# haoheliu/ssr_eval

Hardware: AMD Instinct MI355X
Metric: utterance-pairs/sec (LSD+SSIM, 48kHz, n_fft=2048) (higher is better)
Workload: dtype f64

## Files before the change

ssr_eval_amd/csrc/ssr_metrics.h:

```cpp
#pragma once
#include "ssr_stft.h"

#define SSR_SSIM_NT 64
#define SSR_SSIM_MAXCPT 6
#define SSR_SSIM_WIN 7

SSR_HD constexpr int ssr_ssim_strip_out(int cpt) { return SSR_SSIM_NT * cpt; }
SSR_HD int ssr_ssim_pick_cpt(int n_bins) {
  const int outs = n_bins - (SSR_SSIM_WIN - 1);
  if (outs <= SSR_SSIM_NT * 4) {
    int c = (outs + SSR_SSIM_NT - 1) / SSR_SSIM_NT;
    return c < 1 ? 1 : c;
  }
  int best = 4, best_waste = 1 << 30;
  for (int c = 4; c <= SSR_SSIM_MAXCPT; ++c) {
    const int w = SSR_SSIM_NT * c;
    const int waste = ((outs + w - 1) / w) * w - outs;
    if (waste < best_waste) { best_waste = waste; best = c; }
  }
  return best;
}

struct SsrSsimParams {
  const float* x;
  const float* y;
  const int64_t* frame_off;
  const int32_t* n_rows;
  int F;
  int rows_per_tile, n_row_tiles, n_strips;
  double* part;
  int pitch;
  int vi_n;
  int64_t x_plane;
};
SSR_DEV int ssr_ssim_pitch(const SsrSsimParams& p) { return p.pitch ? p.pitch : p.F; }

template <int CPT> struct SsrSsimRegs {
  double cs[CPT + 1][4];
  double s;
  float px[2][4][CPT + 1];
  float ring[SSR_SSIM_WIN][CPT + 1];
  double pxy[CPT], pb[CPT];
  float den[CPT];
};

template <int CPT> SSR_DEV int ssr_ssim_slot(int c) { return (CPT % 2 == 0) ? c + c / CPT : c; }
template <int CPT> SSR_DEV int ssr_ssim_slot_of(int tid, int d) { return (CPT % 2 == 0) ? (CPT + 1) * tid + (d + d / CPT) : CPT * tid + d; }

template <int CPT, bool CONTIG = false> struct SsrSsimLds {
  static constexpr int PW = SSR_SSIM_NT * CPT + 8 + ((CPT % 2 == 0) ? (SSR_SSIM_NT * CPT + 8) / CPT + 1 : 0);
  static constexpr int NQ = CONTIG ? 1 : 4;
  static constexpr int RW = SSR_SSIM_NT * CPT + 8;
  static constexpr size_t ring_bytes() { return CONTIG ? sizeof(float) * SSR_SSIM_WIN * RW : 0; }
  static constexpr size_t bytes() { return ring_bytes() + sizeof(double) * (NQ * PW + SSR_SSIM_NT + 16 + 8); }
  float* yring; double* col; double* sc0; double* sc1; double* res;
  SSR_MEMBER explicit SsrSsimLds(char* base) {
    yring = reinterpret_cast<float*>(base);
    col = reinterpret_cast<double*>(base + ring_bytes());
    sc0 = col + NQ * PW;
    sc1 = sc0 + SSR_SSIM_NT;
    res = sc1 + 16;
  }
};

SSR_DEV void ssr_ld4(const float* p, float* o) {
#ifdef SSR_HOST_EMU
  memcpy(o, p, 16);
#else
  typedef float f4 __attribute__((ext_vector_type(4)));
  const f4 v = *reinterpret_cast<const f4*>(p);
  o[0] = v.x; o[1] = v.y; o[2] = v.z; o[3] = v.w;
#endif
}
SSR_DEV void ssr_st4(float* p, const float* v) {
#ifdef SSR_HOST_EMU
  memcpy(p, v, 16);
#else
  typedef float f4 __attribute__((ext_vector_type(4)));
  *reinterpret_cast<f4*>(p) = f4{v[0], v[1], v[2], v[3]};
#endif
}

struct SsrImage {
#ifdef SSR_HOST_EMU
  const float* base;
  SSR_MEMBER SsrImage(const float* p, int64_t) : base(p) {}
  SSR_MEMBER float at(int64_t row_elems, unsigned col) const { return base[row_elems + col]; }
  SSR_MEMBER void at4(int64_t row_elems, unsigned col, float* o) const { memcpy(o, base + row_elems + col, 16); }
#else
  __amdgpu_buffer_rsrc_t rsrc;
  SSR_MEMBER SsrImage(const float* p, int64_t n_elems)
      : rsrc(__builtin_amdgcn_make_buffer_rsrc((void*)p, 0, (int)(n_elems * 4), 0x00020000)) {}
  SSR_MEMBER float at(int64_t row_elems, unsigned col) const {
    return __builtin_bit_cast(float, __builtin_amdgcn_raw_buffer_load_b32(rsrc, (int)(col * 4u), (int)(row_elems * 4), 0));
  }
  SSR_MEMBER void at4(int64_t row_elems, unsigned col, float* o) const {
    typedef float f4 __attribute__((ext_vector_type(4)));
    const f4 v = __builtin_bit_cast(f4, __builtin_amdgcn_raw_buffer_load_b128(rsrc, (int)(col * 4u), (int)(row_elems * 4), 0));
    o[0] = v.x; o[1] = v.y; o[2] = v.z; o[3] = v.w;
  }
#endif
};

template <int CPT, bool CONTIG> SSR_DEV int ssr_ssim_col(int tid, int i) {
  if constexpr (CONTIG) return (i < CPT) ? CPT * tid + i : SSR_SSIM_NT * CPT + tid;
  else return tid + SSR_SSIM_NT * i;
}

SSR_DEV int ssr_ssim_row_ahead(int row, int T) { return row < T ? row : T - 1; }

template <int CPT, bool CONTIG, int SET>
SSR_DEV void ssr_ssim_row_load(const SsrSsimParams& p, SsrSsimRegs<CPT>& R, int tid, const SsrImage& x, const SsrImage& y,
                               int row_add, int row_sub, int c_in0, int ncol_in) {
  constexpr int VC = CPT + 1;
  const bool sub = row_sub >= 0;
  const int pitch = ssr_ssim_pitch(p);
// ... 34 lines not shown
#pragma unroll
  for (int i = 0; i < VC; ++i) {
    if (ssr_ssim_col<CPT, CONTIG>(tid, i) < ncol_in) {
      const double a = (double)R.px[SET][0][i], b = (double)R.px[SET][1][i];
      const double c = sub ? (double)R.px[SET][2][i] : 0.0, d = sub ? (double)R.px[SET][3][i] : 0.0;
      R.cs[i][0] = (R.cs[i][0] + a) - c;
      R.cs[i][1] = (R.cs[i][1] + b) - d;
      R.cs[i][2] = fma(-d, d, fma(-c, c, fma(b, b, fma(a, a, R.cs[i][2]))));
      R.cs[i][3] = fma(-c, d, fma(a, b, R.cs[i][3]));
    }
  }
}

template <int CPT, int SET, int SLOT>
SSR_DEV void ssr_ssim_row_apply_contig(SsrSsimRegs<CPT>& R, float* yrow, int tid) {
  constexpr int VC = CPT + 1;
  float* own = yrow + CPT * tid;
  float* ext = yrow + SSR_SSIM_NT * CPT + (tid < 7 ? tid : 7);
  float d[VC];
#pragma unroll
  for (int h = 0; h < CPT / 4; ++h) ssr_ld4(own + 4 * h, d + 4 * h);
  d[CPT] = *ext;
#pragma unroll
  for (int h = 0; h < CPT / 4; ++h) ssr_st4(own + 4 * h, R.px[SET][1] + 4 * h);
  *ext = R.px[SET][1][CPT];
#pragma unroll
  for (int i = 0; i < VC; ++i) {
    const double a = (double)R.px[SET][0][i], b = (double)R.px[SET][1][i];
    const double c = (double)R.ring[SLOT][i], dd = (double)d[i];
    R.cs[i][0] = (R.cs[i][0] + a) - c;
    R.cs[i][1] = (R.cs[i][1] + b) - dd;
    R.cs[i][2] = fma(-dd, dd, fma(-c, c, fma(b, b, fma(a, a, R.cs[i][2]))));
    R.cs[i][3] = fma(-c, dd, fma(a, b, R.cs[i][3]));
    R.ring[SLOT][i] = R.px[SET][0][i];
    ssr_touch(R.ring[SLOT][i]);
  }
}

struct SsrSsimK {
  static constexpr double n = 49.0;
  static constexpr float cov = (float)(49.0 / 48.0);
  static constexpr float C1n = (float)((0.01 * 2.0) * (0.01 * 2.0) * 49.0 * 49.0), C2n = (float)((0.03 * 2.0) * (0.03 * 2.0) * 49.0 * 49.0);
};
SSR_DEV void ssr_ssim_stage1(double sx, double sy, double& pxy, double& pp) { pxy = sx * sy; pp = fma(sx, sx, sy * sy); }
SSR_DEV float ssr_ssim_stage2f(double pp, double sq) {
  const double t2 = fma(SsrSsimK::n, sq, -pp);
  const float b1 = (float)pp + SsrSsimK::C1n;
  const float b2 = fmaf(SsrSsimK::cov, (float)t2, SsrSsimK::C2n);
  return b1 * b2;
}
SSR_DEV float ssr_ssim_stage3f(double pxy, double sxy, float b12) {
  const double t1 = fma(SsrSsimK::n, sxy, -pxy);
  const float a1 = fmaf(2.0f, (float)pxy, SsrSsimK::C1n);
  const float a2 = fmaf(2.0f * SsrSsimK::cov, (float)t1, SsrSsimK::C2n);
#ifndef SSR_HOST_EMU
  return (a1 * a2) * __builtin_amdgcn_rcpf(b12);
#else
  return (a1 * a2) / b12;
#endif
}
SSR_DEV double ssr_ssim_value(double sx, double sy, double sq, double sxy) {
  double pxy, pp;
  ssr_ssim_stage1(sx, sy, pxy, pp);
  return (double)ssr_ssim_stage3f(pxy, sxy, ssr_ssim_stage2f(pp, sq));
}

#ifndef SSR_HOST_EMU
#define SSR_SSIM_ST(arr, idx, val) (*(volatile __attribute__((address_space(3))) double*)(&(arr)[idx]) = (val))
#define SSR_SSIM_LD(arr, idx) (*(const volatile __attribute__((address_space(3))) double*)(&(arr)[idx]))
#else
#define SSR_SSIM_ST(arr, idx, val) ((arr)[idx] = (val))
#define SSR_SSIM_LD(arr, idx) ((arr)[idx])
#endif
template <int CPT, bool CONTIG, typename BLK>
SSR_BODY void ssr_ssim_body(const SsrSsimParams& p, BLK& blk, int tile, int item, char* lds_base) {
  constexpr int NT = SSR_SSIM_NT, PW = SsrSsimLds<CPT, CONTIG>::PW, VC = CPT + 1, W = SSR_SSIM_WIN;
  using Regs = SsrSsimRegs<CPT>;
  using Lds = SsrSsimLds<CPT, CONTIG>;
  Lds L(lds_base);
  const int row_tile = tile / p.n_strips, strip = tile % p.n_strips;
  const int item_v = item;
  const float* xbase = p.x;
  if (p.vi_n > 0) { xbase += (int64_t)(item / p.vi_n) * p.x_plane; item = item % p.vi_n; }
  const int T = p.n_rows[item];
  const int out_rows = T - (W - 1);
  const int r0 = row_tile * p.rows_per_tile;
  const int r1 = (r0 + p.rows_per_tile < out_rows) ? r0 + p.rows_per_tile : out_rows;
  const int c_in0 = strip * ssr_ssim_strip_out(CPT);
  const int ncol_in = (p.F - c_in0 < NT * CPT + (W - 1)) ? p.F - c_in0 : NT * CPT + (W - 1);
  const int ncol_out = ncol_in - (W - 1);
  double* part = p.part + (int64_t)item_v * p.n_row_tiles * p.n_strips + tile;
  const int pitch = ssr_ssim_pitch(p);
  const SsrImage x(xbase + p.frame_off[item] * pitch, (int64_t)T * pitch);
  const SsrImage y(p.y + p.frame_off[item] * pitch, (int64_t)T * pitch);

  SSR_REGS(Regs, regs, blk);
  if (r0 >= r1 || ncol_out <= 0) {
    SSR_PHASE(blk, regs, if (tid == 0) *part = 0.0);
    return;
  }
  const int n_steps = (W - 1) + (r1 - r0);
#define SSR_SSIM_STEP(s_, SET, SLOT)                                                                                         \
  SSR_PHASE(blk, regs, {                                                                                                    \
    ssr_ssim_row_apply<CPT, false, SET, SLOT>(R, tid, (s_) >= W, ncol_in);                                                   \
    ssr_ssim_row_load<CPT, false, SET>(p, R, tid, x, y, ssr_ssim_row_ahead(r0 + (s_) + 2, T),                               \
                                       ((s_) + 2 >= W) ? r0 + (s_) + 2 - W : -1, c_in0, ncol_in);                           \
    if ((s_) >= W - 1) {                                                                                                    \
      for (int i = 0; i < VC; ++i) {                                                                                        \
        const int c = ssr_ssim_col<CPT, false>(tid, i);                                                                     \
        if (c < ncol_in)                                                                                                    \
          for (int q = 0; q < 4; ++q) L.col[q * PW + ssr_ssim_slot<CPT>(c)] = R.cs[i][q];                                    \
      }                                                                                                                     \
    }                                                                                                                       \
  });                                                                                                                       \
  if ((s_) >= W - 1) {                                                                                                      \
    SSR_PHASE(blk, regs, {                                                                                                  \
      const int j0 = tid * CPT;                                                                                             \
      if (j0 < ncol_out) {                                                                                                  \
        double w[4][CPT];                                      \
        for (int q = 0; q < 4; ++q) {                                                                                       \
          double v[CPT + W - 1];                                                                                            \
          for (int d = 0; d < CPT + W - 1; ++d) {                                                                           \
            int c = j0 + d;                                                                                                 \
            if (c >= ncol_in) c = ncol_in - 1;                                \
            v[d] = L.col[q * PW + ssr_ssim_slot<CPT>(c)];                                                                   \
          }                                                                                                                 \
          double sw = v[0];                                                                                                 \
          for (int d = 1; d < W; ++d) sw += v[d];                                                                           \
          w[q][0] = sw;                                                                                                     \
          for (int i = 1; i < CPT; ++i) {                                                                                   \
            sw += v[i + W - 1] - v[i - 1];                                                                                  \
            w[q][i] = sw;                                                                                                   \
          }                                                                                                                 \
        }                                                                                                                   \
        for (int i = 0; i < CPT; ++i)                                                                                       \
          if (j0 + i < ncol_out) R.s += ssr_ssim_value(w[0][i], w[1][i], w[2][i], w[3][i]);                                  \
      }                                                                                                                     \
    });                                                                                                                     \
  }
  SSR_PHASE(blk, regs, {
    for (int i = 0; i < VC; ++i)
      for (int q = 0; q < 4; ++q) R.cs[i][q] = 0.0;
    R.s = 0.0;
    if constexpr (CONTIG) {
      const float z4[4] = {0.0f, 0.0f, 0.0f, 0.0f};
      for (int k = 0; k < W; ++k) {
        for (int i = 0; i < VC; ++i) R.ring[k][i] = 0.0f;
        for (int h = 0; h < CPT / 4; ++h) ssr_st4(L.yring + k * Lds::RW + CPT * tid + 4 * h, z4);
        L.yring[k * Lds::RW + NT * CPT + (tid & 7)] = 0.0f;
      }
    }
    ssr_ssim_row_load<CPT, CONTIG, 0>(p, R, tid, x, y, r0, -1, c_in0, ncol_in);
    if (n_steps > 1) ssr_ssim_row_load<CPT, CONTIG, 1>(p, R, tid, x, y, r0 + 1, -1, c_in0, ncol_in);
  });
  if constexpr (CONTIG) {
#define SSR_SSIM_STEP_C(s_, SET, SLOT, HORIZ)                                                                                     \
    SSR_WPHASE(blk, regs, {                                                                                                  \
      ssr_ssim_row_apply_contig<CPT, SET, SLOT>(R, L.yring + (SLOT) * Lds::RW, tid);                                              \
      SSR_SCHED_BARRIER();                                                                                                   \
      ssr_ssim_row_load<CPT, true, SET>(p, R, tid, x, y, ssr_ssim_row_ahead(r0 + (s_) + 2, T), -1, c_in0, ncol_in);          \
      SSR_SCHED_BARRIER();    \
    });                                                                                                                      \
    if (HORIZ) {                                                                                                             \
      SSR_UNROLL for (int q = 0; q < 4; ++q) {                                                                               \
        SSR_WPHASE(blk, regs, {              \
                                \
          SSR_UNROLL for (int i = 0; i < (CPT < 6 ? CPT : 6); ++i) SSR_SSIM_ST(L.col, ssr_ssim_slot_of<CPT>(tid, i), R.cs[i][q]);     \
// ... 51 lines not shown
    } while (0);
#undef SSR_SSIM_STEP_T
#undef SSR_SSIM_STEP_K
#undef SSR_SSIM_STEP_C
  } else {
    for (int s0 = 0; s0 < n_steps; s0 += 2) {
      SSR_SSIM_STEP(s0, 0, 0)
      if (s0 + 1 < n_steps) { SSR_SSIM_STEP(s0 + 1, 1, 0) }
    }
  }
#undef SSR_SSIM_STEP
#define SSR_GET_S(q) R.s
  SSR_BLOCK_SUM(blk, regs, NT, 1, L.sc0, L.sc1, L.res, SSR_GET_S);
#undef SSR_GET_S
  SSR_PHASE(blk, regs, if (tid == 0) *part = L.res[0]);
}

struct SsrSpecRedParams {
  const float* x; const float* y;
  const int64_t* frame_off; const int32_t* n_rows;
  int F, metric_mask, rows_per_chunk, n_chunks;
  double* part;
};
struct SsrSpecRedRegs { double acc[7]; double lsd_sum; };
struct SsrSpecRedLds {
  static constexpr int NT = 256;
  static constexpr size_t bytes() { return sizeof(double) * (NT + 16 + 8); }
  double* sc0; double* sc1; double* res;
  SSR_MEMBER explicit SsrSpecRedLds(char* base) {
    sc0 = reinterpret_cast<double*>(base); sc1 = sc0 + NT; res = sc1 + 16;
  }
};

template <typename BLK>
SSR_BODY void ssr_specred_body(const SsrSpecRedParams& p, BLK& blk, int chunk, int item, char* lds_base) {
  constexpr int NT = SsrSpecRedLds::NT;
  SsrSpecRedLds L(lds_base);
  const int T = p.n_rows[item];
  const int t0 = chunk * p.rows_per_chunk;
  const int t1 = (t0 + p.rows_per_chunk < T) ? t0 + p.rows_per_chunk : T;
  const float* x = p.x + p.frame_off[item] * p.F;
  const float* y = p.y + p.frame_off[item] * p.F;
  double* part = p.part + ((int64_t)item * p.n_chunks + chunk) * SSR_NPART;
  const bool want_lsd = p.metric_mask & SSR_M_LSD;
  SSR_REGS(SsrSpecRedRegs, regs, blk);
  SSR_PHASE(blk, regs, for (int q = 0; q < 7; ++q) R.acc[q] = 0.0; R.lsd_sum = 0.0);
  for (int t = t0; t < t1; ++t) {
    SSR_PHASE(blk, regs, {
      R.acc[0] = 0.0;
      for (int k = tid; k < p.F; k += NT)
        ssr_accumulate_metrics(x[(int64_t)t * p.F + k], y[(int64_t)t * p.F + k], p.metric_mask, R.acc);
      L.sc0[tid] = R.acc[0];
    });
    if (want_lsd) {
      SSR_PHASE(blk, regs, if (tid < 16) {
        double s = 0.0;
        for (int i = tid; i < NT; i += 16) s += L.sc0[i];
        L.sc1[tid] = s;
      });
      SSR_PHASE(blk, regs, if (tid == 0) {
        double s = 0.0;
        for (int i = 0; i < 16; ++i) s += L.sc1[i];
        R.lsd_sum += sqrt(s / (double)p.F);
      });
    }
  }
#define SSR_GET_ACC(q) R.acc[(q) + 1]
  SSR_BLOCK_SUM(blk, regs, NT, 6, L.sc0, L.sc1, L.res, SSR_GET_ACC);
#undef SSR_GET_ACC
  SSR_PHASE(blk, regs, if (tid == 0) {
    part[0] = R.lsd_sum;
    for (int q = 0; q < 6; ++q) part[1 + q] = L.res[q];
    part[7] = 0.0;
  });
}

struct SsrFinalizeParams {
  const double* part; int n_chunks;
  const double* ssim_part; int n_tiles;
  const int32_t* n_rows;
  int F, metric_mask, n_items;
  double* out;
  int vi_n, out_keys, out_key0;
};

SSR_DEV double ssr_sispec_from_sums(double sdd, double stt, double sdt) {
  const double EPS = 1e-12;
  const double den = stt + EPS;
  const double alpha = (stt + sdt) / den;
  const double beta = (EPS - sdt) / den;
  const double tt = alpha * alpha * stt;
  double nn = sdd + 2.0 * beta * sdt + beta * beta * stt;
  if (nn < 0.0) nn = 0.0;
  return 10.0 * log10(tt / (nn + EPS) + EPS);
}

SSR_DEV void ssr_finalize_item(const SsrFinalizeParams& p, int item) {
  const double nan_ = NAN;
  const int real = p.vi_n > 0 ? item % p.vi_n : item;
  double* o = p.vi_n > 0 ? p.out + ((int64_t)real * p.out_keys + p.out_key0 + item / p.vi_n) * 4 : p.out + (int64_t)item * 4;
  const int T = p.n_rows[real];
  o[0] = o[1] = o[2] = o[3] = nan_;
  if (p.part) {
    double s[SSR_NPART];
    for (int q = 0; q < SSR_NPART; ++q) s[q] = 0.0;
    for (int c = 0; c < p.n_chunks; ++c)
      for (int q = 0; q < SSR_NPART; ++q) s[q] += p.part[((int64_t)item * p.n_chunks + c) * SSR_NPART + q];
    if (p.metric_mask & SSR_M_LSD) o[0] = s[0] / (double)T;
    if (p.metric_mask & SSR_M_LOG_SISPEC) o[1] = ssr_sispec_from_sums(s[4], s[5], s[6]);
    if (p.metric_mask & SSR_M_SISPEC) o[2] = ssr_sispec_from_sums(s[1], s[2], s[3]);
  }
  if (p.ssim_part && (p.metric_mask & SSR_M_SSIM)) {
    double s = 0.0;
    for (int c = 0; c < p.n_tiles; ++c) s += p.ssim_part[(int64_t)item * p.n_tiles + c];
    o[3] = (T >= SSR_SSIM_WIN && p.F >= SSR_SSIM_WIN) ? s / ((double)(T - 6) * (double)(p.F - 6)) : nan_;
  }
}
```

ssr_eval_amd/csrc/ssr_specred_wave.h:

```cpp
#pragma once
#include "ssr_stft.h"

struct SsrSpecWaveParams {
  const float* x;
  const float* y;
  const int64_t* frame_off;
  const int32_t* n_rows;
  int F, pitch, metric_mask, rows_per_chunk, n_chunks, vi_n;
  int64_t x_plane;
  double* part;
};

struct SsrSpecTgt2 { f2 t, tt, lt; };

__device__ __forceinline__ SsrSpecTgt2 ssr_spec_tgt2(float t0, float t1) {
  const f2 t = f2_make(t0, t1);
  return {t, t * t, ssr_log10f_fast2(t + f2_splat(1e-12f))};
}
__device__ __forceinline__ void ssr_spec_tgt_sums2(const SsrSpecTgt2& y, double* tsum) {
  const double t0 = (double)y.t.x, l0 = (double)y.lt.x, t1 = (double)y.t.y, l1 = (double)y.lt.y;
  tsum[0] += t0 * t0; tsum[1] += l0 * l0;
  tsum[0] += t1 * t1; tsum[1] += l1 * l1;
}
__device__ __forceinline__ void ssr_spec_est2(float e0, float e1, const SsrSpecTgt2& y, double* acc) {
  const f2 EPS2 = f2_splat(1e-12f);
  const f2 e = f2_make(e0, e1);
  const f2 ee = e + EPS2;
  const f2 d = ssr_log10f_fast2(ssr_divf_fast2(y.tt, ee * ee) + EPS2);
  const f2 dd = d * d;
  const f2 le = ssr_log10f_fast2(ee);
  {
    acc[0] += (double)dd.x;
    const double td = (double)y.t.x, d0 = (double)e.x - td;
    acc[1] += d0 * d0; acc[3] += d0 * td;
    const double ld = (double)y.lt.x, l0 = (double)le.x - ld;
    acc[4] += l0 * l0; acc[6] += l0 * ld;
  }
  {
    acc[0] += (double)dd.y;
    const double td = (double)y.t.y, d0 = (double)e.y - td;
    acc[1] += d0 * d0; acc[3] += d0 * td;
    const double ld = (double)y.lt.y, l0 = (double)le.y - ld;
    acc[4] += l0 * l0; acc[6] += l0 * ld;
  }
}

template <int KG>
__device__ __forceinline__ void ssr_specred_wave_body(const SsrSpecWaveParams& p, int chunk, int group_v) {
  const int lane = (int)threadIdx.x;
  const int key0 = (group_v / p.vi_n) * KG, item = group_v % p.vi_n;
  const int T = p.n_rows[item];
  const int t0 = chunk * p.rows_per_chunk;
  const int t1 = (t0 + p.rows_per_chunk < T) ? t0 + p.rows_per_chunk : T;
  const float* x = p.x + (int64_t)key0 * p.x_plane + p.frame_off[item] * (int64_t)p.pitch;
  const float* y = p.y + p.frame_off[item] * (int64_t)p.pitch;
  const int mask = p.metric_mask;
  const bool want_lsd = mask & SSR_M_LSD;
  constexpr int FULL = SSR_M_LSD | SSR_M_SISPEC | SSR_M_LOG_SISPEC;
  const bool fast = (mask & FULL) == FULL;
  double acc[KG][7];
  double lsd_sum[KG];
  double tsum[2] = {0.0, 0.0};
#pragma unroll
  for (int g = 0; g < KG; ++g) {
    lsd_sum[g] = 0.0;
#pragma unroll
    for (int q = 0; q < 7; ++q) acc[g][q] = 0.0;
  }
  const int nq = (p.F + 3) / 4;
  const int nfull = p.F / 4;
  for (int t = t0; t < t1; ++t) {
    const float4* yr = reinterpret_cast<const float4*>(y + (int64_t)t * p.pitch);
#pragma unroll
    for (int g = 0; g < KG; ++g) acc[g][0] = 0.0;
    if (fast) {
      for (int q = lane; q < nfull; q += 64) {
        const float4 yv = yr[q];
        float4 xv[KG];
#pragma unroll
        for (int g = 0; g < KG; ++g) xv[g] = reinterpret_cast<const float4*>(x + (int64_t)g * p.x_plane + (int64_t)t * p.pitch)[q];
        const SsrSpecTgt2 y01 = ssr_spec_tgt2(yv.x, yv.y), y23 = ssr_spec_tgt2(yv.z, yv.w);
        ssr_spec_tgt_sums2(y01, tsum);
        ssr_spec_tgt_sums2(y23, tsum);
#pragma unroll
        for (int g = 0; g < KG; ++g) {
          ssr_spec_est2(xv[g].x, xv[g].y, y01, acc[g]);
          ssr_spec_est2(xv[g].z, xv[g].w, y23, acc[g]);
        }
      }
      if (nfull < nq && lane == nfull % 64) {
        const float4 yv = yr[nfull];
        const int k = 4 * nfull;
        double a7[7];
#pragma unroll
        for (int g = 0; g < KG; ++g) {
          const float4 xv = reinterpret_cast<const float4*>(x + (int64_t)g * p.x_plane + (int64_t)t * p.pitch)[nfull];
          a7[0] = acc[g][0]; a7[1] = acc[g][1]; a7[2] = tsum[0]; a7[3] = acc[g][3]; a7[4] = acc[g][4]; a7[5] = tsum[1]; a7[6] = acc[g][6];
          ssr_accumulate_metrics<true>(xv.x, yv.x, mask, a7);
          if (k + 1 < p.F) ssr_accumulate_metrics<true>(xv.y, yv.y, mask, a7);
          if (k + 2 < p.F) ssr_accumulate_metrics<true>(xv.z, yv.z, mask, a7);
          acc[g][0] = a7[0]; acc[g][1] = a7[1]; acc[g][3] = a7[3]; acc[g][4] = a7[4]; acc[g][6] = a7[6];
          if (g == KG - 1) { tsum[0] = a7[2]; tsum[1] = a7[5]; }
        }
      }
    } else {
      for (int q = lane; q < nq; q += 64) {
        const float4 yv = yr[q];
        const int k = 4 * q;
#pragma unroll
        for (int g = 0; g < KG; ++g) {
          const float4 xv = reinterpret_cast<const float4*>(x + (int64_t)g * p.x_plane + (int64_t)t * p.pitch)[q];
          ssr_accumulate_metrics<true>(xv.x, yv.x, mask, acc[g]);
          if (k + 1 < p.F) ssr_accumulate_metrics<true>(xv.y, yv.y, mask, acc[g]);
          if (k + 2 < p.F) ssr_accumulate_metrics<true>(xv.z, yv.z, mask, acc[g]);
          if (k + 3 < p.F) ssr_accumulate_metrics<true>(xv.w, yv.w, mask, acc[g]);
        }
      }
    }
    if (want_lsd) {
#pragma unroll
      for (int g = 0; g < KG; ++g) lsd_sum[g] += sqrt(ssr_wave_sum<64>(acc[g][0]) / (double)p.F);
    }
  }
  if (fast) {
#pragma unroll
    for (int g = 0; g < KG; ++g) { acc[g][2] = tsum[0]; acc[g][5] = tsum[1]; }
  }
#pragma unroll
  for (int g = 0; g < KG; ++g) {
    double tot[6];
#pragma unroll
    for (int q = 0; q < 6; ++q) tot[q] = ssr_wave_sum<64>(acc[g][1 + q]);
    if (lane == 0) {
      double* part = p.part + (((int64_t)(key0 + g) * p.vi_n + item) * p.n_chunks + chunk) * SSR_NPART;
// ... 8 lines not shown
```

ssr_eval_amd/csrc/tu_metrics.hip:

```cpp
#include "ssr_host.h"
#include "ssr_metrics.h"
#include "ssr_pair_transform.h"

template <int CPT, bool CONTIG>
__global__ __launch_bounds__(SSR_SSIM_NT, (CPT == 8 ? 2 : 1)) void k_ssim(SsrSsimParams p) {
  extern __shared__ __attribute__((aligned(16))) char smem[];
  SsrBlk blk{(int)threadIdx.x};
  const int tiles = p.n_row_tiles * p.n_strips;
  ssr_ssim_body<CPT, CONTIG>(p, blk, blockIdx.x % tiles, blockIdx.x / tiles, smem);
}


__global__ __launch_bounds__(256) void k_specred(SsrSpecRedParams p) {
  extern __shared__ __attribute__((aligned(16))) char smem[];
  SsrBlk blk{(int)threadIdx.x};
  ssr_specred_body(p, blk, blockIdx.x % p.n_chunks, blockIdx.x / p.n_chunks, smem);
}

__global__ __launch_bounds__(64) void k_finalize(SsrFinalizeParams p) {
  const int item = blockIdx.x * 64 + threadIdx.x;
  if (item < p.n_items) ssr_finalize_item(p, item);
}

struct SsimGeom { int rows_per_tile, n_row_tiles, n_strips, cpt; };
static SsimGeom ssim_geom(int max_rows, int n_bins, int n_items, bool aligned_rows) {
  SsimGeom g;
  const int out_rows = max_rows - 6 > 1 ? max_rows - 6 : 1;
  int64_t r = ((int64_t)out_rows * n_items + ssr_target_wgs() - 1) / ssr_target_wgs();
  if (r < 8) r = 8;
  if (r > 128) r = 128;
  if (r > out_rows) r = out_rows;
  g.rows_per_tile = (int)r;
  g.n_row_tiles = ssr_ceil_div(out_rows, g.rows_per_tile);
  g.cpt = ssr_ssim_pick_cpt(n_bins);
  if (aligned_rows && g.cpt != 4) {
    const int outs = n_bins - (SSR_SSIM_WIN - 1);
    if (outs > 0) {
      const int strips4 = ssr_ceil_div(outs, ssr_ssim_strip_out(4)), strips_c = ssr_ceil_div(outs, ssr_ssim_strip_out(g.cpt));
      if (strips4 * 5 * 68 < strips_c * (g.cpt + 1) * 100) g.cpt = 4;
    }
  }
  if (aligned_rows && g.cpt == 4) {
    constexpr int SSR_SSIM_TRIP4 = 3731, SSR_SSIM_TRIP8 = 6371;
    const int outs = n_bins - (SSR_SSIM_WIN - 1);
    if (outs > 0 && ssr_ceil_div(outs, ssr_ssim_strip_out(8)) * SSR_SSIM_TRIP8 < ssr_ceil_div(outs, ssr_ssim_strip_out(4)) * SSR_SSIM_TRIP4)
      g.cpt = 8;
  }
  g.n_strips = n_bins > 6 ? ssr_ceil_div(n_bins - 6, ssr_ssim_strip_out(g.cpt)) : 1;
  return g;
}


struct PairWs {
  SsrPairGeom g;
  SsimGeom sg;
  SsrPairImages im;
  size_t off_part, off_ssim, total;
};
static PairWs pair_ws(const ssr_plan* pl, int n_items, int max_len, int64_t total_rows, bool in64, bool want_mag) {
  PairWs w;
  w.g = ssr_pair_geom(pl, n_items, max_len, in64);
  w.sg = ssim_geom((int)ssr_num_frames(pl, max_len), pl->n_bins, n_items, true);
  w.im = ssr_pair_images_layout(pl, 1, total_rows, in64, want_mag);
  size_t o = w.im.end;
  w.off_part = o; o += ssr_align256((size_t)n_items * w.g.n_chunks * SSR_NPART * sizeof(double));
  w.off_ssim = o; o += ssr_align256((size_t)n_items * w.sg.n_row_tiles * w.sg.n_strips * sizeof(double));
  w.total = o;
  return w;
}

extern "C" size_t ssr_pair_metrics_workspace_bytes_for(const ssr_plan* pl, int n_items, int max_len, int64_t total_rows,
                                                        unsigned metric_mask) {
  if (!pl || n_items <= 0) return 0;
  const bool mag = metric_mask & SSR_METRIC_SSIM;
  const size_t a = pair_ws(pl, n_items, max_len, total_rows, false, mag).total, b = pair_ws(pl, n_items, max_len, total_rows, true, mag).total;
  return (a > b ? a : b) + ssr_align256((size_t)n_items * sizeof(int32_t));
}

extern "C" size_t ssr_pair_metrics_workspace_bytes(const ssr_plan* pl, int n_items, int max_len, int64_t total_rows) {
  return ssr_pair_metrics_workspace_bytes_for(pl, n_items, max_len, total_rows, SSR_METRIC_ALL);
}

template <int CPT, bool CONTIG = false> static int launch_ssim_inst(const SsrSsimParams& p, int grid, hipStream_t s) {
  const size_t lds = SsrSsimLds<CPT, CONTIG>::bytes();
  static thread_local SsrLdsSlot slot;
  if (int rc = ssr_allow_lds((const void*)k_ssim<CPT, CONTIG>, lds, &slot)) return rc;
  hipLaunchKernelGGL((k_ssim<CPT, CONTIG>), dim3(grid), dim3(SSR_SSIM_NT), lds, s, p);
  HIP_TRY(hipGetLastError());
  return SSR_OK;
}

static int launch_ssim(const float* x, const float* y, const int64_t* frame_off, const int32_t* n_rows, int n_items,
                       int F, int pitch, const SsimGeom& g, double* part, hipStream_t s, int vi_n = 0, int64_t x_plane = 0) {
  SsrSsimParams p{x, y, frame_off, n_rows, F, g.rows_per_tile, g.n_row_tiles, g.n_strips, part, pitch, vi_n, x_plane};
  const int grid = n_items * g.n_row_tiles * g.n_strips;
  const bool contig = pitch > 0 && pitch % 4 == 0 && (((uintptr_t)x | (uintptr_t)y) & 15) == 0;
  if (g.cpt == 8) {
    if (!contig) return ssr_fail(SSR_ERR_UNSUPPORTED, "eight-column SSIM geometry on unaligned rows");
    return launch_ssim_inst<8, true>(p, grid, s);
  }
  if (g.cpt == 4 && contig) return launch_ssim_inst<4, true>(p, grid, s);
  switch (g.cpt) {
    case 1: return launch_ssim_inst<1>(p, grid, s);
    case 2: return launch_ssim_inst<2>(p, grid, s);
    case 3: return launch_ssim_inst<3>(p, grid, s);
    case 4: return launch_ssim_inst<4>(p, grid, s);
    case 5: return launch_ssim_inst<5>(p, grid, s);
    case 6: return launch_ssim_inst<6>(p, grid, s);
  }
  return ssr_fail(SSR_ERR_UNSUPPORTED, "bad SSIM geometry");
}

static int launch_finalize(const double* part, int n_chunks, const double* ssim_part, int n_tiles, const int32_t* n_rows,
                           int F, unsigned mask, int n_items, double* out, hipStream_t s) {
  SsrFinalizeParams p{part, n_chunks, ssim_part, n_tiles, n_rows, F, (int)mask, n_items, out};
  hipLaunchKernelGGL(k_finalize, dim3(ssr_ceil_div(n_items, 64)), dim3(64), 0, s, p);
  HIP_TRY(hipGetLastError());
  return SSR_OK;
}

__global__ void k_rows_from_len(const int32_t* len, int n_items, int n_fft, int hop, int32_t* rows) {
  const int i = blockIdx.x * 256 + threadIdx.x;
  if (i < n_items) rows[i] = ssr_num_frames_dev(len[i], n_fft, hop);
}
int ssr_launch_rows_from_len(const ssr_plan* pl, const int32_t* len, int n_items, int32_t* rows, hipStream_t s) {
  hipLaunchKernelGGL(k_rows_from_len, dim3(ssr_ceil_div(n_items, 256)), dim3(256), 0, s, len, n_items, pl->n_fft, pl->hop, rows);
  HIP_TRY(hipGetLastError());
  return SSR_OK;
}

static int pair_metrics_impl(const ssr_plan* pl, const float* est, const double* est64, const int64_t* est_off,
                             const float* tgt, const double* tgt64, const int64_t* tgt_off, const int32_t* len, const int64_t* frame_off,
                             int n_items, int max_len, int64_t total_rows, unsigned mask, double* out,
                             void* workspace, size_t workspace_bytes, void* stream, int stages) {
  int max_T;
  if (int rc = ssr_check_pair_batch(pl, (est || est64) && (tgt || tgt64) && est_off && tgt_off && len && frame_off && out, n_items, 1, max_len,
                                    mask & SSR_METRIC_SSIM, &max_T))
    return rc;
  if (!max_T) return SSR_OK;
  if ((mask & ~SSR_METRIC_ALL) || mask == 0) return ssr_fail(SSR_ERR_INVALID_ARG, "bad metric mask");
  const bool want_ssim = mask & SSR_METRIC_SSIM;
  if (want_ssim && (max_T < 7 || pl->n_bins < 7)) return ssr_fail(SSR_ERR_INVALID_ARG, "win_size exceeds image extent");
  const PairWs w = pair_ws(pl, n_items, max_len, total_rows, est64 != nullptr, want_ssim);
  const size_t rows_bytes = ssr_align256((size_t)n_items * sizeof(int32_t));
  if (!workspace || workspace_bytes < w.total + rows_bytes) return ssr_fail(SSR_ERR_WORKSPACE, "workspace too small");
  char* ws = (char*)workspace;
  int32_t* rows = (int32_t*)(ws + w.total);
  float *est_plane = (float*)(ws + w.im.off_est), *tgt_plane = (float*)(ws + w.im.off_tgt);
  hipStream_t s = (hipStream_t)stream;
  int rc = SSR_OK;
  if (stages & 1) {
    if ((rc = ssr_launch_rows_from_len(pl, len, n_items, rows, s))) return rc;
    rc = ssr_pair_transform(pl, {len, frame_off, n_items, w.g},
                            {est, est64, est_off, tgt, tgt64, tgt_off, mask, want_ssim ? SSR_OUT_MAG : SSR_OUT_NONE, est_plane, tgt_plane,
                             (double*)(ws + w.off_part)}, s);
    if (rc) return rc;
  }
  if ((stages & 2) && want_ssim) {
    rc = launch_ssim(est_plane, tgt_plane, frame_off, rows, n_items, pl->n_bins, ssr_mag_pitch(pl->n_bins), w.sg, (double*)(ws + w.off_ssim), s);
    if (rc) return rc;
  }
  if (stages & 4) {
    rc = launch_finalize((const double*)(ws + w.off_part), w.g.n_chunks, want_ssim ? (const double*)(ws + w.off_ssim) : nullptr,
                         w.sg.n_row_tiles * w.sg.n_strips, rows, pl->n_bins, mask, n_items, out, s);
  }
  return rc;
}

extern "C" int ssr_pair_metrics_stages(const ssr_plan* pl, const float* est, const int64_t* est_off, const float* tgt,
                                       const int64_t* tgt_off, const int32_t* len, const int64_t* frame_off,
                                       int n_items, int max_len, int64_t total_rows, unsigned mask, double* out,
                                       void* workspace, size_t workspace_bytes, void* stream, int stages) {
  return pair_metrics_impl(pl, est, nullptr, est_off, tgt, nullptr, tgt_off, len, frame_off, n_items, max_len, total_rows,
                           mask, out, workspace, workspace_bytes, stream, stages);
}

extern "C" int ssr_pair_metrics(const ssr_plan* pl, const float* est, const int64_t* est_off, const float* tgt,
                                const int64_t* tgt_off, const int32_t* len, const int64_t* frame_off, int n_items,
                                int max_len, int64_t total_rows, unsigned mask, double* out, void* workspace,
                                size_t workspace_bytes, void* stream) {
  return pair_metrics_impl(pl, est, nullptr, est_off, tgt, nullptr, tgt_off, len, frame_off, n_items, max_len, total_rows,
                           mask, out, workspace, workspace_bytes, stream, 7);
}

extern "C" int ssr_pair_metrics_est64(const ssr_plan* pl, const double* est, const int64_t* est_off, const float* tgt,
                                      const int64_t* tgt_off, const int32_t* len, const int64_t* frame_off, int n_items,
                                      int max_len, int64_t total_rows, unsigned mask, double* out, void* workspace,
                                      size_t workspace_bytes, void* stream) {
  return pair_metrics_impl(pl, nullptr, est, est_off, tgt, nullptr, tgt_off, len, frame_off, n_items, max_len, total_rows,
                           mask, out, workspace, workspace_bytes, stream, 7);
}

extern "C" int ssr_pair_metrics_f64(const ssr_plan* pl, const double* est, const int64_t* est_off, const double* tgt,
                                    const int64_t* tgt_off, const int32_t* len, const int64_t* frame_off, int n_items,
                                    int max_len, int64_t total_rows, unsigned mask, double* out, void* workspace,
                                    size_t workspace_bytes, void* stream) {
  return pair_metrics_impl(pl, nullptr, est, est_off, nullptr, tgt, tgt_off, len, frame_off, n_items, max_len, total_rows,
                           mask, out, workspace, workspace_bytes, stream, 7);
}

#include "ssr_specred_wave.h"
template <int KG> __global__ __launch_bounds__(64) void k_specred_wave(SsrSpecWaveParams p) {
  ssr_specred_wave_body<KG>(p, blockIdx.x % p.n_chunks, blockIdx.x / p.n_chunks);
}

struct MultiWs {
  SsrPairGeom g;
  SsimGeom sg;
  SsrPairImages im;
  size_t off_part_a, off_part_s, off_ssim, off_rows, total;
  int spec_rows_per_chunk, spec_chunks, spec_kg, n_tiles;
  bool fast;
};
static MultiWs multi_ws(const ssr_plan* pl, int n_items, int n_keys, int max_len, int64_t total_rows, unsigned mask, bool est64 = false) {
  MultiWs m;
  const bool want_ssim = mask & SSR_METRIC_SSIM;
  m.fast = ssr_multi_fast_path(pl, est64) && n_keys > 1;
  m.g = ssr_pair_geom(pl, n_items, max_len, est64);
  const int max_T = (int)ssr_num_frames(pl, max_len);
  m.sg = ssim_geom(max_T, pl->n_bins, m.fast ? n_items * n_keys : n_items, true);
  m.n_tiles = m.sg.n_row_tiles * m.sg.n_strips;
  m.im = ssr_pair_images_layout(pl, n_keys, total_rows, est64, want_ssim || m.fast, false);
  const int n_spec = ((n_keys - 1) / 2) * 2;
  m.spec_kg = ssr_keys_per_wave(n_spec);
  m.spec_rows_per_chunk = ssr_wave_rows_per_wg(max_T, (int64_t)n_items * (n_spec > 0 ? n_spec / m.spec_kg : 1));
  m.spec_chunks = ssr_ceil_div(max_T, m.spec_rows_per_chunk);
  size_t o = m.im.end;
  m.off_part_a = o; o += 2 * ssr_align256((size_t)n_items * m.g.n_chunks * SSR_NPART * sizeof(double));
  m.off_part_s = o; o += ssr_align256((size_t)n_items * n_keys * m.spec_chunks * SSR_NPART * sizeof(double));
  m.off_ssim = o; o += ssr_align256((size_t)n_items * n_keys * m.n_tiles * sizeof(double));
  m.off_rows = o; o += ssr_align256((size_t)n_items * sizeof(int32_t));
  m.total = o;
  return m;
}

extern "C" size_t ssr_pair_metrics_multi_workspace_bytes(const ssr_plan* pl, int n_items, int n_keys, int max_len, int64_t total_rows,
                                                         unsigned metric_mask) {
  if (!pl || n_items <= 0 || n_keys <= 0) return 0;
  return multi_ws(pl, n_items, n_keys, max_len, total_rows, metric_mask).total;
}

static int pair_metrics_multi_impl(const ssr_plan* pl, const float* est, const double* est64, const int64_t* est_off, const float* tgt,
                                   const int64_t* tgt_off, const int32_t* len, const int64_t* frame_off, int n_items, int n_keys, int max_len,
                                   int64_t total_rows, unsigned mask, double* out, void* workspace, size_t workspace_bytes, void* stream) {
  int max_T;
  if (int rc = ssr_check_pair_batch(pl, (est || est64) && est_off && tgt && tgt_off && len && frame_off && out, n_items, n_keys, max_len, true,
                                    &max_T))
    return rc;
  if (!max_T) return SSR_OK;
  if ((mask & ~SSR_METRIC_ALL) || mask == 0) return ssr_fail(SSR_ERR_INVALID_ARG, "bad metric mask");
  const bool want_ssim = mask & SSR_METRIC_SSIM;
  if (want_ssim && (max_T < 7 || pl->n_bins < 7)) return ssr_fail(SSR_ERR_INVALID_ARG, "win_size exceeds image extent");
  const MultiWs m = multi_ws(pl, n_items, n_keys, max_len, total_rows, mask, est64 != nullptr);
  if (!workspace || workspace_bytes < m.total) return ssr_fail(SSR_ERR_WORKSPACE, "workspace too small");
  char* ws = (char*)workspace;
  hipStream_t s = (hipStream_t)stream;
  int32_t* rows = (int32_t*)(ws + m.off_rows);
  int rc;
  if ((rc = ssr_launch_rows_from_len(pl, len, n_items, rows, s))) return rc;
  const SsrPairBatch bt{len, frame_off, n_items, m.g};
  const bool mag = m.im.plane != 0;
  const int pitch = ssr_mag_pitch(pl->n_bins);
  const int64_t plane_floats = (int64_t)(m.im.plane / sizeof(float));
  const unsigned red_mask = mask & (SSR_METRIC_LSD | SSR_METRIC_LOG_SISPEC | SSR_METRIC_SISPEC);
  auto plane_of = [&](int k) { return mag ? (float*)(ws + m.im.off_est + (size_t)k * m.im.plane) : nullptr; };
  float* tgt_plane = mag ? (float*)(ws + m.im.off_tgt) : nullptr;
  double* part0 = (double*)(ws + m.off_part_a);
  double* ssim_part = (double*)(ws + m.off_ssim);
  auto finalize = [&](const double* part, int n_chunks, const double* sp, int n_virtual, int key0) {
    SsrFinalizeParams p{part, n_chunks, want_ssim ? sp : nullptr, m.n_tiles, rows, pl->n_bins, (int)mask, n_virtual, out, n_items, n_keys, key0};
    hipLaunchKernelGGL(k_finalize, dim3(ssr_ceil_div(n_virtual, 64)), dim3(64), 0, s, p);
    return hipGetLastError();
  };
  auto ssim = [&](int key0, int n_k) {
    return launch_ssim(plane_of(key0), tgt_plane, frame_off, rows, n_items * n_k, pl->n_bins, pitch, m.sg,
                       ssim_part + (size_t)key0 * n_items * m.n_tiles, s, n_items, plane_floats);
  };
  if (!m.fast) {
    for (int k = 0; k < n_keys; ++k) {
      rc = ssr_pair_transform(pl, bt, {est, est64, est_off + (size_t)k * n_items, tgt, nullptr, tgt_off, mask, mag ? SSR_OUT_MAG : SSR_OUT_NONE,
                                       plane_of(k), tgt_plane, part0}, s);
      if (rc) return rc;
      if (want_ssim && (rc = ssim(k, 1))) return rc;
      HIP_TRY(finalize(part0, m.g.n_chunks, ssim_part + (size_t)k * n_items * m.n_tiles, n_items, k));
    }
    return SSR_OK;
  }
  const int n_spec = ((n_keys - 1) / 2) * 2;
  const int k_last = n_spec + 1;
  const bool odd_last = k_last < n_keys;
  double* part_last = (double*)(ws + m.off_part_a + ssr_align256((size_t)n_items * m.g.n_chunks * SSR_NPART * sizeof(double)));
  if ((rc = ssr_pair_images(pl, bt, est, est64, est_off, tgt, tgt_off, n_keys, m.im, ws, s, mask, part0, part_last))) return rc;
  if (n_spec > 0 && red_mask) {
    SsrSpecWaveParams q{plane_of(1), tgt_plane, frame_off, rows, pl->n_bins, pitch, (int)red_mask, m.spec_rows_per_chunk, m.spec_chunks, n_items,
                        plane_floats, (double*)(ws + m.off_part_s)};
    const int kg = m.spec_kg;
    const dim3 grid((unsigned)((int64_t)(n_spec / kg) * n_items * m.spec_chunks));
    if (kg == 3) hipLaunchKernelGGL(k_specred_wave<3>, grid, dim3(64), 0, s, q);
    else if (kg == 2) hipLaunchKernelGGL(k_specred_wave<2>, grid, dim3(64), 0, s, q);
    else hipLaunchKernelGGL(k_specred_wave<1>, grid, dim3(64), 0, s, q);
    HIP_TRY(hipGetLastError());
  }
  if (want_ssim && (rc = ssim(0, n_keys))) return rc;
  HIP_TRY(finalize(part0, m.g.n_chunks, ssim_part, n_items, 0));
  if (n_spec > 0)
    HIP_TRY(finalize(red_mask ? (const double*)(ws + m.off_part_s) : nullptr, m.spec_chunks, ssim_part + (size_t)n_items * m.n_tiles, n_spec * n_items, 1));
  if (odd_last) HIP_TRY(finalize(part_last, m.g.n_chunks, ssim_part + (size_t)k_last * n_items * m.n_tiles, n_items, k_last));
  return SSR_OK;
}

extern "C" int ssr_pair_metrics_multi(const ssr_plan* pl, const float* est, const int64_t* est_off, const float* tgt, const int64_t* tgt_off,
                                      const int32_t* len, const int64_t* frame_off, int n_items, int n_keys, int max_len, int64_t total_rows,
                                      unsigned mask, double* out, void* workspace, size_t workspace_bytes, void* stream) {
  if (!est) return ssr_fail(SSR_ERR_INVALID_ARG, "null argument");
  return pair_metrics_multi_impl(pl, est, nullptr, est_off, tgt, tgt_off, len, frame_off, n_items, n_keys, max_len, total_rows, mask, out,
                                 workspace, workspace_bytes, stream);
}

extern "C" size_t ssr_pair_metrics_multi_est64_workspace_bytes(const ssr_plan* pl, int n_items, int n_keys, int max_len, int64_t total_rows,
                                                               unsigned metric_mask) {
  if (!pl || n_items <= 0 || n_keys <= 0) return 0;
  return multi_ws(pl, n_items, n_keys, max_len, total_rows, metric_mask, true).total;
}
extern "C" int ssr_pair_metrics_multi_est64(const ssr_plan* pl, const double* est, const int64_t* est_off, const float* tgt, const int64_t* tgt_off,
                                            const int32_t* len, const int64_t* frame_off, int n_items, int n_keys, int max_len,
                                            int64_t total_rows, unsigned mask, double* out, void* workspace, size_t workspace_bytes,
                                            void* stream) {
  if (!est) return ssr_fail(SSR_ERR_INVALID_ARG, "null argument");
  return pair_metrics_multi_impl(pl, nullptr, est, est_off, tgt, tgt_off, len, frame_off, n_items, n_keys, max_len, total_rows, mask, out,
                                 workspace, workspace_bytes, stream);
}

struct SpecWs { size_t off_part, off_ssim, total; int rows_per_chunk, n_chunks; SsimGeom sg; };
static SpecWs spec_ws(int n_items, int max_rows, int n_bins) {
  SpecWs w;
  w.rows_per_chunk = ssr_units_per_chunk_for(max_rows, n_items);
  w.n_chunks = ssr_ceil_div(max_rows, w.rows_per_chunk);
  w.sg = ssim_geom(max_rows, n_bins, n_items, false);
  size_t o = 0;
  w.off_part = o; o += ssr_align256((size_t)n_items * w.n_chunks * SSR_NPART * sizeof(double));
  w.off_ssim = o; o += ssr_align256((size_t)n_items * w.sg.n_row_tiles * w.sg.n_strips * sizeof(double));
  w.total = o;
  return w;
}

extern "C" size_t ssr_spectrogram_metrics_workspace_bytes(int n_items, int max_rows, int n_bins) {
  if (n_items <= 0) return 0;
  return spec_ws(n_items, max_rows, n_bins).total;
}

extern "C" int ssr_spectrogram_metrics(const float* est_sp, const float* tgt_sp, const int64_t* frame_off,
                                       const int32_t* n_rows, int n_items, int max_rows, int n_bins, unsigned mask,
                                       double* out, void* workspace, size_t workspace_bytes, void* stream) {
  if (!est_sp || !tgt_sp || !frame_off || !n_rows || !out) return ssr_fail(SSR_ERR_INVALID_ARG, "null argument");
  if (n_items <= 0) return SSR_OK;
  if ((mask & ~SSR_METRIC_ALL) || mask == 0) return ssr_fail(SSR_ERR_INVALID_ARG, "bad metric mask");
  if (max_rows < 1 || n_bins < 1) return ssr_fail(SSR_ERR_INVALID_ARG, "empty spectrogram");
  if ((int64_t)max_rows * n_bins >= ((int64_t)1 << 30))
    return ssr_fail(SSR_ERR_UNSUPPORTED, "spectrogram of 2^30 elements or more (4 GiB buffer views)");
  const bool want_ssim = mask & SSR_METRIC_SSIM;
  if (want_ssim && (max_rows < 7 || n_bins < 7)) return ssr_fail(SSR_ERR_INVALID_ARG, "win_size exceeds image extent");
  const SpecWs w = spec_ws(n_items, max_rows, n_bins);
  if (!workspace || workspace_bytes < w.total) return ssr_fail(SSR_ERR_WORKSPACE, "workspace too small");
  char* ws = (char*)workspace;
  hipStream_t s = (hipStream_t)stream;
  const bool want_red = mask & (SSR_METRIC_LSD | SSR_METRIC_SISPEC | SSR_METRIC_LOG_SISPEC);
  if (want_red) {
    SsrSpecRedParams p{est_sp, tgt_sp, frame_off, n_rows, n_bins, (int)mask, w.rows_per_chunk, w.n_chunks,
                       (double*)(ws + w.off_part)};
    hipLaunchKernelGGL(k_specred, dim3(n_items * w.n_chunks), dim3(256), SsrSpecRedLds::bytes(), s, p);
    HIP_TRY(hipGetLastError());
  }
  if (want_ssim) {
    int rc = launch_ssim(est_sp, tgt_sp, frame_off, n_rows, n_items, n_bins, 0, w.sg, (double*)(ws + w.off_ssim), s);
    if (rc) return rc;
  }
  return launch_finalize(want_red ? (const double*)(ws + w.off_part) : nullptr, w.n_chunks,
                         want_ssim ? (const double*)(ws + w.off_ssim) : nullptr, w.sg.n_row_tiles * w.sg.n_strips, n_rows,
                         n_bins, mask, n_items, out, s);
}
```

Baseline: 374,900.

## Compute frame counts inline from lengths and schedule SSIM tiles newest-first

Drops the separate rows-from-length kernel launch and its workspace buffer. The SSIM, spectral-reduction and finalize kernels now derive each item's frame count on the fly from the raw lengths and the plan's n_fft/hop. The SSIM grid in the pair paths is also traversed in reverse item order, so tiles whose spectrogram planes were written most recently are processed first, presumably to reuse data still in cache. The cost is a small per-block recomputation of the frame count and a slightly more complex parameter plumbing.

```diff
diff --git a/ssr_eval_amd/csrc/ssr_metrics.h b/ssr_eval_amd/csrc/ssr_metrics.h
--- a/ssr_eval_amd/csrc/ssr_metrics.h
+++ b/ssr_eval_amd/csrc/ssr_metrics.h
@@ -19,6 +19,10 @@
     if (waste < best_waste) { best_waste = waste; best = c; }
   }
   return best;
+}
+
+SSR_DEV int ssr_rows_of(const int32_t* n_rows, int item, int len_n_fft, int len_hop) {
+  return len_n_fft > 0 ? ssr_num_frames_dev(n_rows[item], len_n_fft, len_hop) : n_rows[item];
 }
 
 struct SsrSsimParams {
@@ -32,6 +36,8 @@
   int pitch;
   int vi_n;
   int64_t x_plane;
+  int len_n_fft, len_hop;
+  int newest_first;
 };
 SSR_DEV int ssr_ssim_pitch(const SsrSsimParams& p) { return p.pitch ? p.pitch : p.F; }
 
@@ -232,7 +238,7 @@
   const int item_v = item;
   const float* xbase = p.x;
   if (p.vi_n > 0) { xbase += (int64_t)(item / p.vi_n) * p.x_plane; item = item % p.vi_n; }
-  const int T = p.n_rows[item];
+  const int T = ssr_rows_of(p.n_rows, item, p.len_n_fft, p.len_hop);
   const int out_rows = T - (W - 1);
   const int r0 = row_tile * p.rows_per_tile;
   const int r1 = (r0 + p.rows_per_tile < out_rows) ? r0 + p.rows_per_tile : out_rows;
@@ -450,6 +456,7 @@
   int F, metric_mask, n_items;
   double* out;
   int vi_n, out_keys, out_key0;
+  int len_n_fft, len_hop;
 };
 
 SSR_DEV double ssr_sispec_from_sums(double sdd, double stt, double sdt) {
@@ -467,7 +474,7 @@
   const double nan_ = NAN;
   const int real = p.vi_n > 0 ? item % p.vi_n : item;
   double* o = p.vi_n > 0 ? p.out + ((int64_t)real * p.out_keys + p.out_key0 + item / p.vi_n) * 4 : p.out + (int64_t)item * 4;
-  const int T = p.n_rows[real];
+  const int T = ssr_rows_of(p.n_rows, real, p.len_n_fft, p.len_hop);
   o[0] = o[1] = o[2] = o[3] = nan_;
   if (p.part) {
     double s[SSR_NPART];
diff --git a/ssr_eval_amd/csrc/ssr_specred_wave.h b/ssr_eval_amd/csrc/ssr_specred_wave.h
--- a/ssr_eval_amd/csrc/ssr_specred_wave.h
+++ b/ssr_eval_amd/csrc/ssr_specred_wave.h
@@ -1,5 +1,5 @@
 #pragma once
-#include "ssr_stft.h"
+#include "ssr_metrics.h"
 
 struct SsrSpecWaveParams {
   const float* x;
@@ -9,6 +9,7 @@
   int F, pitch, metric_mask, rows_per_chunk, n_chunks, vi_n;
   int64_t x_plane;
   double* part;
+  int len_n_fft, len_hop;
 };
 
 struct SsrSpecTgt2 { f2 t, tt, lt; };
@@ -49,7 +50,7 @@
 __device__ __forceinline__ void ssr_specred_wave_body(const SsrSpecWaveParams& p, int chunk, int group_v) {
   const int lane = (int)threadIdx.x;
   const int key0 = (group_v / p.vi_n) * KG, item = group_v % p.vi_n;
-  const int T = p.n_rows[item];
+  const int T = ssr_rows_of(p.n_rows, item, p.len_n_fft, p.len_hop);
   const int t0 = chunk * p.rows_per_chunk;
   const int t1 = (t0 + p.rows_per_chunk < T) ? t0 + p.rows_per_chunk : T;
   const float* x = p.x + (int64_t)key0 * p.x_plane + p.frame_off[item] * (int64_t)p.pitch;
diff --git a/ssr_eval_amd/csrc/tu_metrics.hip b/ssr_eval_amd/csrc/tu_metrics.hip
--- a/ssr_eval_amd/csrc/tu_metrics.hip
+++ b/ssr_eval_amd/csrc/tu_metrics.hip
@@ -7,7 +7,8 @@
   extern __shared__ __attribute__((aligned(16))) char smem[];
   SsrBlk blk{(int)threadIdx.x};
   const int tiles = p.n_row_tiles * p.n_strips;
-  ssr_ssim_body<CPT, CONTIG>(p, blk, blockIdx.x % tiles, blockIdx.x / tiles, smem);
+  const int slot = blockIdx.x / tiles;
+  ssr_ssim_body<CPT, CONTIG>(p, blk, blockIdx.x % tiles, p.newest_first ? (int)(gridDim.x / tiles) - 1 - slot : slot, smem);
 }
 
 
@@ -74,7 +75,7 @@
   if (!pl || n_items <= 0) return 0;
   const bool mag = metric_mask & SSR_METRIC_SSIM;
   const size_t a = pair_ws(pl, n_items, max_len, total_rows, false, mag).total, b = pair_ws(pl, n_items, max_len, total_rows, true, mag).total;
-  return (a > b ? a : b) + ssr_align256((size_t)n_items * sizeof(int32_t));
+  return a > b ? a : b;
 }
 
 extern "C" size_t ssr_pair_metrics_workspace_bytes(const ssr_plan* pl, int n_items, int max_len, int64_t total_rows) {
@@ -90,9 +91,14 @@
   return SSR_OK;
 }
 
-static int launch_ssim(const float* x, const float* y, const int64_t* frame_off, const int32_t* n_rows, int n_items,
-                       int F, int pitch, const SsimGeom& g, double* part, hipStream_t s, int vi_n = 0, int64_t x_plane = 0) {
-  SsrSsimParams p{x, y, frame_off, n_rows, F, g.rows_per_tile, g.n_row_tiles, g.n_strips, part, pitch, vi_n, x_plane};
+struct RowCounts { const int32_t* v; int n_fft, hop; };
+static RowCounts rows_given(const int32_t* n_rows) { return {n_rows, 0, 0}; }
+static RowCounts rows_from_len(const ssr_plan* pl, const int32_t* len) { return {len, pl->n_fft, pl->hop}; }
+
+static int launch_ssim(const float* x, const float* y, const int64_t* frame_off, const RowCounts& rows, int n_items,
+                       int F, int pitch, const SsimGeom& g, double* part, hipStream_t s, bool newest_first, int vi_n = 0, int64_t x_plane = 0) {
+  SsrSsimParams p{x, y, frame_off, rows.v, F, g.rows_per_tile, g.n_row_tiles, g.n_strips, part, pitch, vi_n, x_plane, rows.n_fft, rows.hop,
+                  newest_first ? 1 : 0};
   const int grid = n_items * g.n_row_tiles * g.n_strips;
   const bool contig = pitch > 0 && pitch % 4 == 0 && (((uintptr_t)x | (uintptr_t)y) & 15) == 0;
   if (g.cpt == 8) {
@@ -111,9 +117,9 @@
   return ssr_fail(SSR_ERR_UNSUPPORTED, "bad SSIM geometry");
 }
 
-static int launch_finalize(const double* part, int n_chunks, const double* ssim_part, int n_tiles, const int32_t* n_rows,
+static int launch_finalize(const double* part, int n_chunks, const double* ssim_part, int n_tiles, const RowCounts& rows,
                            int F, unsigned mask, int n_items, double* out, hipStream_t s) {
-  SsrFinalizeParams p{part, n_chunks, ssim_part, n_tiles, n_rows, F, (int)mask, n_items, out};
+  SsrFinalizeParams p{part, n_chunks, ssim_part, n_tiles, rows.v, F, (int)mask, n_items, out, 0, 0, 0, rows.n_fft, rows.hop};
   hipLaunchKernelGGL(k_finalize, dim3(ssr_ceil_div(n_items, 64)), dim3(64), 0, s, p);
   HIP_TRY(hipGetLastError());
   return SSR_OK;
@@ -142,22 +148,20 @@
   const bool want_ssim = mask & SSR_METRIC_SSIM;
   if (want_ssim && (max_T < 7 || pl->n_bins < 7)) return ssr_fail(SSR_ERR_INVALID_ARG, "win_size exceeds image extent");
   const PairWs w = pair_ws(pl, n_items, max_len, total_rows, est64 != nullptr, want_ssim);
-  const size_t rows_bytes = ssr_align256((size_t)n_items * sizeof(int32_t));
-  if (!workspace || workspace_bytes < w.total + rows_bytes) return ssr_fail(SSR_ERR_WORKSPACE, "workspace too small");
+  if (!workspace || workspace_bytes < w.total) return ssr_fail(SSR_ERR_WORKSPACE, "workspace too small");
   char* ws = (char*)workspace;
-  int32_t* rows = (int32_t*)(ws + w.total);
+  const RowCounts rows = rows_from_len(pl, len);
   float *est_plane = (float*)(ws + w.im.off_est), *tgt_plane = (float*)(ws + w.im.off_tgt);
   hipStream_t s = (hipStream_t)stream;
   int rc = SSR_OK;
   if (stages & 1) {
-    if ((rc = ssr_launch_rows_from_len(pl, len, n_items, rows, s))) return rc;
     rc = ssr_pair_transform(pl, {len, frame_off, n_items, w.g},
                             {est, est64, est_off, tgt, tgt64, tgt_off, mask, want_ssim ? SSR_OUT_MAG : SSR_OUT_NONE, est_plane, tgt_plane,
                              (double*)(ws + w.off_part)}, s);
     if (rc) return rc;
   }
   if ((stages & 2) && want_ssim) {
-    rc = launch_ssim(est_plane, tgt_plane, frame_off, rows, n_items, pl->n_bins, ssr_mag_pitch(pl->n_bins), w.sg, (double*)(ws + w.off_ssim), s);
+    rc = launch_ssim(est_plane, tgt_plane, frame_off, rows, n_items, pl->n_bins, ssr_mag_pitch(pl->n_bins), w.sg, (double*)(ws + w.off_ssim), s, true);
     if (rc) return rc;
   }
   if (stages & 4) {
@@ -208,7 +212,7 @@
   SsrPairGeom g;
   SsimGeom sg;
   SsrPairImages im;
-  size_t off_part_a, off_part_s, off_ssim, off_rows, total;
+  size_t off_part_a, off_part_s, off_ssim, total;
   int spec_rows_per_chunk, spec_chunks, spec_kg, n_tiles;
   bool fast;
 };
@@ -229,7 +233,6 @@
   m.off_part_a = o; o += 2 * ssr_align256((size_t)n_items * m.g.n_chunks * SSR_NPART * sizeof(double));
   m.off_part_s = o; o += ssr_align256((size_t)n_items * n_keys * m.spec_chunks * SSR_NPART * sizeof(double));
   m.off_ssim = o; o += ssr_align256((size_t)n_items * n_keys * m.n_tiles * sizeof(double));
-  m.off_rows = o; o += ssr_align256((size_t)n_items * sizeof(int32_t));
   m.total = o;
   return m;
 }
@@ -255,9 +258,8 @@
   if (!workspace || workspace_bytes < m.total) return ssr_fail(SSR_ERR_WORKSPACE, "workspace too small");
   char* ws = (char*)workspace;
   hipStream_t s = (hipStream_t)stream;
-  int32_t* rows = (int32_t*)(ws + m.off_rows);
+  const RowCounts rows = rows_from_len(pl, len);
   int rc;
-  if ((rc = ssr_launch_rows_from_len(pl, len, n_items, rows, s))) return rc;
   const SsrPairBatch bt{len, frame_off, n_items, m.g};
   const bool mag = m.im.plane != 0;
   const int pitch = ssr_mag_pitch(pl->n_bins);
@@ -268,13 +270,14 @@
   double* part0 = (double*)(ws + m.off_part_a);
   double* ssim_part = (double*)(ws + m.off_ssim);
   auto finalize = [&](const double* part, int n_chunks, const double* sp, int n_virtual, int key0) {
-    SsrFinalizeParams p{part, n_chunks, want_ssim ? sp : nullptr, m.n_tiles, rows, pl->n_bins, (int)mask, n_virtual, out, n_items, n_keys, key0};
+    SsrFinalizeParams p{part, n_chunks, want_ssim ? sp : nullptr, m.n_tiles, rows.v, pl->n_bins, (int)mask, n_virtual, out, n_items, n_keys, key0,
+                        rows.n_fft, rows.hop};
     hipLaunchKernelGGL(k_finalize, dim3(ssr_ceil_div(n_virtual, 64)), dim3(64), 0, s, p);
     return hipGetLastError();
   };
   auto ssim = [&](int key0, int n_k) {
     return launch_ssim(plane_of(key0), tgt_plane, frame_off, rows, n_items * n_k, pl->n_bins, pitch, m.sg,
-                       ssim_part + (size_t)key0 * n_items * m.n_tiles, s, n_items, plane_floats);
+                       ssim_part + (size_t)key0 * n_items * m.n_tiles, s, true, n_items, plane_floats);
   };
   if (!m.fast) {
     for (int k = 0; k < n_keys; ++k) {
@@ -292,8 +295,8 @@
   double* part_last = (double*)(ws + m.off_part_a + ssr_align256((size_t)n_items * m.g.n_chunks * SSR_NPART * sizeof(double)));
   if ((rc = ssr_pair_images(pl, bt, est, est64, est_off, tgt, tgt_off, n_keys, m.im, ws, s, mask, part0, part_last))) return rc;
   if (n_spec > 0 && red_mask) {
-    SsrSpecWaveParams q{plane_of(1), tgt_plane, frame_off, rows, pl->n_bins, pitch, (int)red_mask, m.spec_rows_per_chunk, m.spec_chunks, n_items,
-                        plane_floats, (double*)(ws + m.off_part_s)};
+    SsrSpecWaveParams q{plane_of(1), tgt_plane, frame_off, rows.v, pl->n_bins, pitch, (int)red_mask, m.spec_rows_per_chunk, m.spec_chunks, n_items,
+                        plane_floats, (double*)(ws + m.off_part_s), rows.n_fft, rows.hop};
     const int kg = m.spec_kg;
     const dim3 grid((unsigned)((int64_t)(n_spec / kg) * n_items * m.spec_chunks));
     if (kg == 3) hipLaunchKernelGGL(k_specred_wave<3>, grid, dim3(64), 0, s, q);
@@ -372,10 +375,10 @@
     HIP_TRY(hipGetLastError());
   }
   if (want_ssim) {
-    int rc = launch_ssim(est_sp, tgt_sp, frame_off, n_rows, n_items, n_bins, 0, w.sg, (double*)(ws + w.off_ssim), s);
+    int rc = launch_ssim(est_sp, tgt_sp, frame_off, rows_given(n_rows), n_items, n_bins, 0, w.sg, (double*)(ws + w.off_ssim), s, false);
     if (rc) return rc;
   }
   return launch_finalize(want_red ? (const double*)(ws + w.off_part) : nullptr, w.n_chunks,
-                         want_ssim ? (const double*)(ws + w.off_ssim) : nullptr, w.sg.n_row_tiles * w.sg.n_strips, n_rows,
+                         want_ssim ? (const double*)(ws + w.off_ssim) : nullptr, w.sg.n_row_tiles * w.sg.n_strips, rows_given(n_rows),
                          n_bins, mask, n_items, out, s);
 }
```

New measurement: 374,500 (median of 3 runs). Within noise of the previous version (-0.1%).
